# zhangxiaochen95/uav_bs_ctrl

Hardware: AMD Instinct MI355X
Metric: env-steps/sec (MADRQN, 8 UBS x 80 GT) (higher is better)
Workload: dtype f32

## Files before the change

### include/uavgnn.h

```cpp
#ifndef UAVGNN_H
#define UAVGNN_H

#include <stddef.h>
#include <stdint.h>

#ifdef __cplusplus
extern "C" {
#endif

#define UAVGNN_VERSION 100

#define UAVGNN_EINVAL (-1000)
#define UAVGNN_EUNSUPPORTED (-1001)
#define UAVGNN_EWORKSPACE (-1002)

typedef void* uavgnn_stream_t;

int uavgnn_version(void);

const char* uavgnn_strerror(int code);

int uavgnn_gatv2_fwd(const float* x_src, int E, int F_src, const float* x_dst, int F_dst, const int32_t* seg_off,
                     const int32_t* dst_order, int N, const float* W_s, const float* b_s, const float* W_d, const float* b_d, const float* attn,
                     const float* W_r, const float* b_r, int nh, int D, float slope, float* out, int ld_out,
// ... 72 lines not shown
                       int32_t* deg_near, uavgnn_stream_t stream);
int uavgnn_obs_compact(const float* gt, int M, int Fg, const float* ubs, int U, int Fu, int N, const int32_t* seen_off,
                       const int32_t* near_off, float* x_gt, float* x_ubs, uavgnn_stream_t stream);
int uavgnn_talk_degrees(const float* d_u2u, int n, int B, float r_comm, int32_t* deg_in, int32_t* env_edges,
                        uavgnn_stream_t stream);
int uavgnn_talk_compact(const float* d_u2u, int n, int B, float r_comm, const int32_t* talk_off,
                        const int32_t* env_base, int32_t* talk_src, int32_t* talk_eid, uavgnn_stream_t stream);
int uavgnn_offsets_scan4(const int32_t* d0, int n0, int32_t* o0, const int32_t* d1, int n1, int32_t* o1, const int32_t* d2,
                         int n2, int32_t* o2, const int32_t* d3, int n3, int32_t* o3, uavgnn_stream_t stream);

int uavgnn_eps_greedy(const float* q, int ld_q, int N, int A, int n_agents, const float* u_team, const float* u_agent,
                      float eps, long long* acts, uavgnn_stream_t stream);
int uavgnn_eps_greedy_dev(const float* q, int ld_q, int N, int A, int n_agents, const float* u_team, const float* u_agent,
                          const float* eps_dev, long long* acts, uavgnn_stream_t stream);

int uavgnn_colsum_acc(const float* x, long long ld, int N, int C, float* acc, int S, uavgnn_stream_t stream);
int uavgnn_gemm_h2_supported(int M, int N, int K);
long long uavgnn_split_h2_bytes(int n_out, int K);
int uavgnn_split_h2(const float* W, int ld, int R, int C, int transpose, void* planes, uavgnn_stream_t stream);
int uavgnn_gemm_nt_h2(const float* X, int ldx, int K1, const float* X2, int ldx2, int M, int K, const float* rowmax, const float* rowmax2,
                      const void* planes, int N, const float* bias, float* Y, int ldy, int epilogue, uavgnn_stream_t stream);
int uavgnn_gemm_nt_h2_rm2(const float* X, int ldx, int K1, const float* X2, int ldx2, int M, int K, const float* rowmax, float* rowmax2_out,
                          const void* planes, int N, const float* bias, float* Y, int ldy, int epilogue, uavgnn_stream_t stream);
int uavgnn_gru_gates_bwd_fused_sums_rowmax(const float* pre, const float* h, const float* d_hout, const float* dq, int n_out,
                                           const float* W_out, int N, int H, float* d_gi, float* d_gh, float* d_h, float* col_sums,
                                           float* row_absmax, uavgnn_stream_t stream);
int uavgnn_relu_bwd_colsum_rowmax(const float* dy, long long ld, const float* y, long long ldy, float* out, long long ldo, int N, int C,
                                  float* acc, int S, float* row_absmax, uavgnn_stream_t stream);
int uavgnn_relu_bwd_colsum(const float* dy, long long ld, const float* y, long long ldy, float* out, long long ldo, int N, int C,
                           float* acc, int S, uavgnn_stream_t stream);

int uavgnn_flat_obs_supported(int H_out, int F);
int uavgnn_flat_obs_fwd(const float* agent, long long ld_a, int F_a, const float* gt, long long ld_g, int K_g, const float* ubs,
                        long long ld_u, int K_u, int rows, const float* W, const float* b, int H_out, float* y, long long ld_y,
                        uavgnn_stream_t stream);
int uavgnn_flat_obs_wgrad_chunks(long long rows, int H_out, int F);
int uavgnn_flat_obs_wgrad(const float* dy, long long ld_dy, int H_out, const float* agent, long long ld_a, int F_a, const float* gt,
                          long long ld_g, int K_g, const float* ubs, long long ld_u, int K_u, int rows, float* partials, int S,
                          int accumulate, uavgnn_stream_t stream);

int uavgnn_talk_attn_env_supported(int n_max, int M, int K);
int uavgnn_talk_attn_env_fwd(const float* s, int ld_s, const float* q, int ld_q, const float* v, int ld_v, int K, int M,
                             const int32_t* talk_off, const int32_t* talk_src, const int32_t* graph_off, int B,
                             int n_max, float scale, float* c, int ld_c, float* a_save, const float* x_copy, int ld_x,
                             int n_copy, uavgnn_stream_t stream);
int uavgnn_talk_attn_env_bwd(const float* s, int ld_s, const float* q, int ld_q, const float* v, int ld_v, int K, int M,
// ... 123 lines not shown
```

### uav_bs_ctrl_amd/_lib.py

```python
from __future__ import annotations

import ctypes
import os

import torch as th

_HERE = os.path.dirname(os.path.abspath(__file__))
LIB_PATH = os.environ.get("UAVGNN_LIB") or os.path.join(_HERE, "csrc", "libuavgnn.so")

_c_fp = ctypes.c_void_p
_c_ip = ctypes.c_void_p
_c_int = ctypes.c_int
_c_f32 = ctypes.c_float
_c_st = ctypes.c_void_p

SIGNATURES = {
    "uavgnn_version": (_c_int, []),
    "uavgnn_strerror": (ctypes.c_char_p, [_c_int]),
    "uavgnn_gatv2_fwd": (_c_int, [_c_fp, _c_int, _c_int, _c_fp, _c_int, _c_ip, _c_ip, _c_int, _c_fp, _c_fp, _c_fp, _c_fp, _c_fp,
                                  _c_fp, _c_fp, _c_int, _c_int, _c_f32, _c_fp, _c_int, _c_fp, _c_st]),
    "uavgnn_gatv2_fwd_valu": (_c_int, [_c_fp, _c_int, _c_int, _c_fp, _c_int, _c_ip, _c_ip, _c_int, _c_fp, _c_fp, _c_fp, _c_fp, _c_fp,
                                       _c_fp, _c_fp, _c_int, _c_int, _c_f32, _c_fp, _c_int, _c_fp, _c_st]),
    "uavgnn_gatv2_fwd_mfma": (_c_int, [_c_fp, _c_int, _c_int, _c_fp, _c_int, _c_ip, _c_ip, _c_int, _c_fp, _c_fp, _c_fp, _c_fp, _c_fp,
                                       _c_fp, _c_fp, _c_int, _c_int, _c_f32, _c_fp, _c_int, _c_fp, _c_st]),
# ... 68 lines not shown
    "uavgnn_relu_bwd_colsum": (_c_int, [_c_fp, ctypes.c_longlong, _c_fp, ctypes.c_longlong, _c_fp, ctypes.c_longlong, _c_int, _c_int, _c_fp,
                               _c_int, _c_st]),
    "uavgnn_relu_bwd_colsum_rowmax": (_c_int, [_c_fp, ctypes.c_longlong, _c_fp, ctypes.c_longlong, _c_fp, ctypes.c_longlong, _c_int, _c_int,
                                               _c_fp, _c_int, _c_fp, _c_st]),
    "uavgnn_flat_obs_supported": (_c_int, [_c_int, _c_int]),
    "uavgnn_flat_obs_fwd": (_c_int, [_c_fp, ctypes.c_longlong, _c_int, _c_fp, ctypes.c_longlong, _c_int, _c_fp, ctypes.c_longlong, _c_int,
                                     _c_int, _c_fp, _c_fp, _c_int, _c_fp, ctypes.c_longlong, _c_st]),
    "uavgnn_flat_obs_wgrad_chunks": (_c_int, [ctypes.c_longlong, _c_int, _c_int]),
    "uavgnn_flat_obs_wgrad": (_c_int, [_c_fp, ctypes.c_longlong, _c_int, _c_fp, ctypes.c_longlong, _c_int, _c_fp, ctypes.c_longlong, _c_int,
                                       _c_fp, ctypes.c_longlong, _c_int, _c_int, _c_fp, _c_int, _c_int, _c_st]),
    "uavgnn_gemm_nt_x3_rowmax": (_c_int, [_c_fp, _c_int, _c_int, _c_int, ctypes.c_void_p, _c_int, _c_fp, _c_fp, _c_int, _c_int, _c_fp, _c_st]),
    "uavgnn_col_absmax": (_c_int, [_c_fp, ctypes.c_longlong, ctypes.c_longlong, _c_int, _c_fp, _c_st]),
    "uavgnn_gemm_tn_h2_supported": (_c_int, [ctypes.c_longlong, _c_int, _c_int]),
    "uavgnn_gemm_tn_h2_chunks": (_c_int, [ctypes.c_longlong, _c_int, _c_int]),
    "uavgnn_gemm_tn_h2": (_c_int, [_c_fp, ctypes.c_longlong, _c_int, _c_fp, ctypes.c_longlong, _c_int, ctypes.c_longlong, _c_fp, _c_fp, _c_fp,
                                   _c_int, _c_int, _c_st]),
    "uavgnn_gemm_h2_supported": (_c_int, [_c_int, _c_int, _c_int]),
    "uavgnn_split_h2_bytes": (ctypes.c_longlong, [_c_int, _c_int]),
    "uavgnn_split_h2": (_c_int, [_c_fp, _c_int, _c_int, _c_int, _c_int, ctypes.c_void_p, _c_st]),
    "uavgnn_gemm_nt_h2": (_c_int, [_c_fp, _c_int, _c_int, _c_fp, _c_int, _c_int, _c_int, _c_fp, _c_fp, ctypes.c_void_p, _c_int, _c_fp, _c_fp,
                                   _c_int, _c_int, _c_st]),
    "uavgnn_gemm_nt_h2_rm2": (_c_int, [_c_fp, _c_int, _c_int, _c_fp, _c_int, _c_int, _c_int, _c_fp, _c_fp, ctypes.c_void_p, _c_int, _c_fp, _c_fp,
                                       _c_int, _c_int, _c_st]),
    "uavgnn_env_state_dim": (_c_int, [_c_int, _c_int, _c_int]),
    "uavgnn_env_step": (_c_int, [ctypes.POINTER(ctypes.c_int32), ctypes.POINTER(ctypes.c_double), _c_int] + [_c_fp] * 22 + [_c_st]),
    "uavgnn_adamw_polyak": (_c_int, [_c_fp, _c_fp, _c_fp, _c_fp, _c_fp, ctypes.c_longlong, ctypes.c_longlong, _c_fp, ctypes.c_double,
                                     ctypes.c_double, _c_f32, _c_f32, _c_f32, _c_f32, _c_st]),
    "uavgnn_gru_cell_supported": (_c_int, [_c_int, _c_int]),
    "uavgnn_gru_cell_fwd": (_c_int, [_c_fp, _c_int, _c_int, _c_fp, _c_int, _c_int, _c_fp, _c_fp, _c_fp, _c_fp, _c_fp, _c_fp, _c_st]),
    "uavgnn_gru_cell_x3_supported": (_c_int, [_c_int, _c_int]),
    "uavgnn_gru_cell_x3_workspace_bytes": (ctypes.c_longlong, [_c_int, _c_int]),
    "uavgnn_gru_split_weights": (_c_int, [_c_fp, _c_int, _c_fp, _c_int, ctypes.c_void_p, _c_st]),
    "uavgnn_gru_cell_fwd_x3": (_c_int, [_c_fp, _c_int, _c_int, _c_fp, _c_int, _c_int, ctypes.c_void_p, _c_fp, _c_fp, _c_fp, _c_fp, _c_st]),
    "uavgnn_gru_cell_fwd_x3_cat": (_c_int, [_c_fp, _c_int, _c_int, _c_fp, _c_int, _c_int, _c_fp, _c_int, _c_int, ctypes.c_void_p, _c_fp, _c_fp,
                                            _c_fp, _c_fp, _c_st]),
    "uavgnn_gru_cell_fwd_x3_opts": (_c_int, [_c_fp, _c_int, _c_int, _c_fp, _c_int, _c_int, _c_fp, _c_int, _c_int, ctypes.c_void_p, _c_fp, _c_fp,
                                             _c_fp, _c_fp, _c_int, _c_st]),
    "uavgnn_gru_cell_h2_supported": (_c_int, [_c_int, _c_int]),
    "uavgnn_gru_cell_h2_workspace_bytes": (ctypes.c_longlong, [_c_int, _c_int]),
    "uavgnn_gru_split_weights_h2": (_c_int, [_c_fp, _c_int, _c_fp, _c_int, ctypes.c_void_p, _c_st]),
    "uavgnn_gru_cell_fwd_h2": (_c_int, [_c_fp, _c_int, _c_int, _c_fp, _c_int, _c_int, _c_fp, _c_int, _c_int, _c_fp, ctypes.c_void_p, _c_fp,
                                        _c_fp, _c_fp, _c_fp, _c_st]),
    "uavgnn_row_absmax": (_c_int, [_c_fp, _c_int, _c_int, _c_fp, _c_int, _c_int, _c_fp, _c_int, _c_int, _c_int, _c_fp, _c_st]),
    "uavgnn_tarmac_msg_rowmax_supported": (_c_int, [_c_int, _c_int, _c_int, _c_int]),
    "uavgnn_tarmac_msg_fwd_rowmax": (_c_int, [_c_fp, _c_int, _c_fp, _c_int, _c_int, _c_int, _c_int, ctypes.c_void_p, _c_fp, _c_int, _c_int,
                                              _c_ip, _c_ip, _c_f32, _c_fp, _c_int, _c_fp, _c_fp, _c_int, _c_fp, _c_int, _c_fp, _c_st]),
# ... 95 lines not shown
```

### uav_bs_ctrl_amd/csrc/gemm_h2.hip

```cpp
#include "common.h"

namespace uavgnn {
namespace {

typedef float f32x2 __attribute__((ext_vector_type(2)));
typedef float f32x16 __attribute__((ext_vector_type(16)));
typedef _Float16 f16x2 __attribute__((ext_vector_type(2)));
typedef _Float16 f16x8 __attribute__((ext_vector_type(8)));
typedef unsigned u32x4 __attribute__((ext_vector_type(4)));
typedef unsigned u32x2 __attribute__((ext_vector_type(2)));

constexpr int BN = 128, BK = 32, BM8 = 256, NT = 512;
constexpr int PA = BM8 * 4, PB = BN * 4;
constexpr int BUF = 2 * PA + 2 * PB;

__device__ __forceinline__ int swz32(int row) { return (row >> 2) & 3; }
__device__ __forceinline__ f16x8 as_frag(u32x4 v) { return __builtin_bit_cast(f16x8, v); }
__device__ __forceinline__ f32x16 mfma32(f16x8 a, f16x8 b, f32x16 c) { return __builtin_amdgcn_mfma_f32_32x32x16_f16(a, b, c, 0, 0, 0); }
__device__ __forceinline__ int scale_exp(float amax) {
  const int e = static_cast<int>((__float_as_uint(amax) >> 23) & 0xffu);
  return max(-126, min(126, 14 - (e - 127)));
}
__device__ __forceinline__ float pow2f(int e) { return __uint_as_float(static_cast<unsigned>(e + 127) << 23); }

// ... 286 lines not shown
    }
    return;
  }
  }
#pragma unroll
  for (int b = 0; b < 2; ++b) {
    const int col = n0 + wn + b * 32 + l32;
    if (col >= N) continue;
    const float bv = bias != nullptr ? bias[col] : 0.f, ci = winv[col];
#pragma unroll
    for (int a = 0; a < 2; ++a)
#pragma unroll
      for (int i = 0; i < 16; ++i) {
        const int lrow = wm + a * 32 + 8 * (i >> 2) + 4 * lh + (i & 3);
        const int row = m0 + lrow;
        if (row < M) {
          float* p = Y + static_cast<size_t>(row) * ldy + col;
          float v = acc[a][b][i] * ci * sInv[lrow] + bv;
          if (ACC) v += *p;
          if (RELU) v = fmaxf(v, 0.f);
          *p = v;
        }
      }
  }
}

}
}

using namespace uavgnn;

extern "C" int uavgnn_gemm_h2_supported(int M, int N, int K) {
  return (M > 0 && N > 0 && K >= BK && K % BK == 0 && static_cast<long long>(M) * K < (1LL << 31) &&
          2LL * N * K < (1LL << 31)) ? 1 : 0;
}

extern "C" long long uavgnn_split_h2_bytes(int n_out, int K) {
  if (n_out <= 0 || K <= 0) return 0;
  return 4LL * n_out * K + 4LL * n_out;
}

extern "C" int uavgnn_split_h2(const float* W, int ld, int R, int C, int transpose, void* planes, uavgnn_stream_t stream) {
  if (!W || !planes || R <= 0 || C <= 0 || ld < C) return UAVGNN_EINVAL;
  const int n_out = transpose ? C : R, K = transpose ? R : C;
  if ((K & 1) || (reinterpret_cast<uintptr_t>(planes) & 15)) return UAVGNN_EUNSUPPORTED;
  unsigned short* p = static_cast<unsigned short*>(planes);
// ... 29 lines not shown
  if (acc && relu) UAVGNN_H2_GEMM(true, true, IL);    \
  else if (acc) UAVGNN_H2_GEMM(true, false, IL);      \
  else if (relu) UAVGNN_H2_GEMM(false, true, IL);     \
  else UAVGNN_H2_GEMM(false, false, IL);
  if (epilogue & UAVGNN_GEMM_STAGING_INTERLEAVED) { UAVGNN_H2_GEMM_IL(true) }
  else { UAVGNN_H2_GEMM_IL(false) }
#undef UAVGNN_H2_GEMM_IL
#undef UAVGNN_H2_GEMM
  return launch_status();
}

extern "C" int uavgnn_gemm_nt_h2(const float* X, int ldx, int K1, const float* X2, int ldx2, int M, int K, const float* rowmax,
                                 const float* rowmax2, const void* planes, int N, const float* bias, float* Y, int ldy, int epilogue,
                                 uavgnn_stream_t stream) {
  return gemm_nt_h2_launch(X, ldx, K1, X2, ldx2, M, K, rowmax, rowmax2, nullptr, planes, N, bias, Y, ldy, epilogue, stream);
}

extern "C" int uavgnn_gemm_nt_h2_rm2(const float* X, int ldx, int K1, const float* X2, int ldx2, int M, int K, const float* rowmax,
                                     float* rowmax2_out, const void* planes, int N, const float* bias, float* Y, int ldy, int epilogue,
                                     uavgnn_stream_t stream) {
  if (!rowmax2_out) return UAVGNN_EINVAL;
  return gemm_nt_h2_launch(X, ldx, K1, X2, ldx2, M, K, rowmax, nullptr, rowmax2_out, planes, N, bias, Y, ldy, epilogue, stream);
}
```

### uav_bs_ctrl_amd/csrc/gru_fused.hip

```cpp
#include "common.h"

namespace uavgnn {
namespace {

typedef float f32x4 __attribute__((ext_vector_type(4)));
constexpr int BM = 128, BJ = 32, BK = 32, ST = 34;

__device__ __forceinline__ float sigmoidf_(float x) { return 1.f / (1.f + expf(-x)); }

template <bool SAVE>
__global__ __launch_bounds__(256, 2) void gru_cell_fwd_kernel(
    const float* __restrict__ inp, int ld_inp, int K1, const float* __restrict__ h, int N, int H,
    const float* __restrict__ W_ih, const float* __restrict__ b_ih, const float* __restrict__ W_hh,
    const float* __restrict__ b_hh, float* __restrict__ h_out, float* __restrict__ pre) {
  __shared__ __attribute__((aligned(16))) float sA[BM * ST];
  __shared__ __attribute__((aligned(16))) float sB[3 * BJ * ST];
  const int tid = threadIdx.x, lane = tid & 63, wave = tid >> 6;
  const int j = lane & 15, g = lane >> 4;
  const int wm = (wave >> 1) * 64, wc = (wave & 1) * 16;
  const int m0 = blockIdx.y * BM, j0 = blockIdx.x * BJ;

  f32x4 acc[4][4];
#pragma unroll
  for (int a = 0; a < 4; ++a)
// ... 99 lines not shown
      const float nn = tanhf(fmaf(rr, ghn, gin));
      float* hp = sA + lrow * ST + wc + j;
      *hp = fmaf(zz, *hp - nn, nn);
      if (SAVE && row < N) {
        float* p = pre + static_cast<size_t>(row) * 4 * H + c;
        p[0] = pr;
        p[H] = pz;
        p[2 * H] = gin;
        p[3 * H] = ghn;
      }
    }
  }
  __syncthreads();
#pragma unroll
  for (int q = 0; q < 4; ++q) {
    const int idx = tid + 256 * q, row = idx >> 3, c4 = idx & 7;
    if (m0 + row < N) {
      const float* p = sA + row * ST + 4 * c4;
      *reinterpret_cast<float4*>(h_out + static_cast<size_t>(m0 + row) * H + j0 + 4 * c4) = make_float4(p[0], p[1], p[2], p[3]);
    }
  }
}

template <bool HEAD, bool SUMS, bool RM = false>
__global__ __launch_bounds__(256) void gru_gates_bwd_fused_kernel(const float* __restrict__ pre, const float* __restrict__ h,
                                                                  const float* __restrict__ d_hout, long long total, int H,
                                                                  float* __restrict__ d_gi, float* __restrict__ d_gh,
                                                                  float* __restrict__ d_h, const float* __restrict__ dq,
                                                                  int n_out, const float* __restrict__ W_out,
                                                                  float* __restrict__ col_sums,
                                                                  float* __restrict__ row_absmax = nullptr) {
  const int HV = H / 4;
  float cs[SUMS ? 16 : 1];
#pragma unroll
  for (int t = 0; t < (SUMS ? 16 : 1); ++t) cs[t] = 0.f;
  for (long long i = blockIdx.x * 256LL + threadIdx.x; i < total; i += gridDim.x * 256LL) {
    const long long row = i / HV;
    const int col = static_cast<int>(i - row * HV) * 4;
    const float* p = pre + row * 4 * H + col;
    const float4 pr = *reinterpret_cast<const float4*>(p), pz = *reinterpret_cast<const float4*>(p + H);
    const float4 gin = *reinterpret_cast<const float4*>(p + 2 * H), ghn = *reinterpret_cast<const float4*>(p + 3 * H);
    const float4 hh = *reinterpret_cast<const float4*>(h + row * H + col);
    float4 dho = d_hout != nullptr ? *reinterpret_cast<const float4*>(d_hout + row * H + col) : make_float4(0.f, 0.f, 0.f, 0.f);
    if constexpr (HEAD) {
      const float* __restrict__ qr = dq + row * n_out;
      for (int a = 0; a < n_out; ++a) {
        const float qa = qr[a];
// ... 5 lines not shown
      }
    }
    const float a_pr[4] = {pr.x, pr.y, pr.z, pr.w}, a_pz[4] = {pz.x, pz.y, pz.z, pz.w};
    const float a_gi[4] = {gin.x, gin.y, gin.z, gin.w}, a_gh[4] = {ghn.x, ghn.y, ghn.z, ghn.w};
    const float a_h[4] = {hh.x, hh.y, hh.z, hh.w}, a_d[4] = {dho.x, dho.y, dho.z, dho.w};
    float dr[4], dz[4], dni[4], dnh[4], dh[4];
#pragma unroll
    for (int t = 0; t < 4; ++t) {
      const float r = sigmoidf_(a_pr[t]), z = sigmoidf_(a_pz[t]);
      const float n = tanhf(fmaf(r, a_gh[t], a_gi[t]));
      const float dn_pre = a_d[t] * (1.f - z) * (1.f - n * n);
      dni[t] = dn_pre;
      dnh[t] = dn_pre * r;
      dr[t] = dn_pre * a_gh[t] * r * (1.f - r);
      dz[t] = a_d[t] * (a_h[t] - n) * z * (1.f - z);
      dh[t] = a_d[t] * z;
      if constexpr (SUMS) {
        cs[t] += dr[t];
        cs[4 + t] += dz[t];
        cs[8 + t] += dni[t];
        cs[12 + t] += dnh[t];
      }
    }
    float* gi = d_gi + row * 3 * H + col;
    float* gh = d_gh + row * 3 * H + col;
    *reinterpret_cast<float4*>(gi) = make_float4(dr[0], dr[1], dr[2], dr[3]);
    *reinterpret_cast<float4*>(gi + H) = make_float4(dz[0], dz[1], dz[2], dz[3]);
    *reinterpret_cast<float4*>(gi + 2 * H) = make_float4(dni[0], dni[1], dni[2], dni[3]);
    *reinterpret_cast<float4*>(gh) = make_float4(dr[0], dr[1], dr[2], dr[3]);
    *reinterpret_cast<float4*>(gh + H) = make_float4(dz[0], dz[1], dz[2], dz[3]);
    *reinterpret_cast<float4*>(gh + 2 * H) = make_float4(dnh[0], dnh[1], dnh[2], dnh[3]);
    *reinterpret_cast<float4*>(d_h + row * H + col) = make_float4(dh[0], dh[1], dh[2], dh[3]);
    if constexpr (RM) {
      float m = 0.f;
#pragma unroll
      for (int t = 0; t < 4; ++t) m = fmaxf(fmaxf(fmaxf(m, fabsf(dr[t])), fmaxf(fabsf(dz[t]), fabsf(dni[t]))), fabsf(dnh[t]));
      m = wave_max(m);
      if ((threadIdx.x & 63) == 0) row_absmax[row] = m;
    }
  }
  if constexpr (SUMS) {
    __shared__ float sS[256 * 17];
#pragma unroll
    for (int t = 0; t < 16; ++t) sS[threadIdx.x * 17 + t] = cs[t];
    __syncthreads();
    if (static_cast<int>(threadIdx.x) < HV) {
      float* out = col_sums + static_cast<size_t>(blockIdx.x) * 4 * H + 4 * threadIdx.x;
#pragma unroll
      for (int gate = 0; gate < 4; ++gate) {
        float v[4];
#pragma unroll
        for (int t = 0; t < 4; ++t) {
          float a = 0.f;
          for (int part = threadIdx.x; part < 256; part += HV) a += sS[part * 17 + 4 * gate + t];
// ... 74 lines not shown
  const long long total = static_cast<long long>(N) * (H / 4);
  const dim3 grid(capped_grid(total, 256)), block(256);
  if (dq != nullptr)
    hipLaunchKernelGGL((gru_gates_bwd_fused_kernel<true, true>), grid, block, 0, static_cast<hipStream_t>(stream), pre, h, d_hout, total, H,
                       d_gi, d_gh, d_h, dq, n_out, W_out, col_sums);
  else
    hipLaunchKernelGGL((gru_gates_bwd_fused_kernel<false, true>), grid, block, 0, static_cast<hipStream_t>(stream), pre, h, d_hout, total, H,
                       d_gi, d_gh, d_h, nullptr, 0, nullptr, col_sums);
  return launch_status();
}

extern "C" int uavgnn_gru_gates_bwd_fused_sums_rowmax(const float* pre, const float* h, const float* d_hout, const float* dq, int n_out,
                                                      const float* W_out, int N, int H, float* d_gi, float* d_gh, float* d_h,
                                                      float* col_sums, float* row_absmax, uavgnn_stream_t stream) {
  if (N < 0 || H <= 0 || !pre || !h || !d_gi || !d_gh || !d_h || !col_sums || !row_absmax || (dq == nullptr) != (W_out == nullptr) ||
      (dq == nullptr && d_hout == nullptr) || (dq != nullptr && n_out <= 0))
    return UAVGNN_EINVAL;
  if (N == 0) return 0;
  if (H != 256 || !uavgnn_gru_gates_bwd_sum_rows(N, H) || n_out > 64 ||
      ((reinterpret_cast<uintptr_t>(W_out) | reinterpret_cast<uintptr_t>(col_sums)) & 15))
    return UAVGNN_EUNSUPPORTED;
  const long long total = static_cast<long long>(N) * (H / 4);
  const dim3 grid(capped_grid(total, 256)), block(256);
  if (dq != nullptr)
    hipLaunchKernelGGL((gru_gates_bwd_fused_kernel<true, true, true>), grid, block, 0, static_cast<hipStream_t>(stream), pre, h, d_hout, total,
                       H, d_gi, d_gh, d_h, dq, n_out, W_out, col_sums, row_absmax);
  else
    hipLaunchKernelGGL((gru_gates_bwd_fused_kernel<false, true, true>), grid, block, 0, static_cast<hipStream_t>(stream), pre, h, d_hout,
                       total, H, d_gi, d_gh, d_h, nullptr, 0, nullptr, col_sums, row_absmax);
  return launch_status();
}
```

### uav_bs_ctrl_amd/ops.py

```python
from __future__ import annotations

import os
import torch as th

from . import _lib as L

NEG_SLOPE = 0.2
K1_IMAGE = os.environ.get("UAVGNN_K1_IMAGE", "1") != "0"
HETERO_FUSED = True
K1_BF16Z = os.environ.get("UAVGNN_K1_BF16Z", "1") != "0"
K1_ROWMAX = os.environ.get("UAVGNN_K1_ROWMAX", "1") != "0"
K1_ROWMAX_MIN_ROWS = 1 << 17
GEMM_H2_RM2 = os.environ.get("UAVGNN_GEMM_H2_RM2", "1") != "0"
K1_ROWMAX_DENSE_DEG = int(os.environ.get("UAVGNN_K1_ROWMAX_DENSE_DEG", "16"))
K1_ROWMAX_DENSE_MIN_ROWS = 16384


class _KernelTimer:

    def __init__(self):
        self.enabled = False
        self.only = None
        self._spans = {}

# ... 628 lines not shown
            L.check(lib.uavgnn_split_h2(Wc.data_ptr(), n_out, K, n_out, 1, p.data_ptr(), L.stream()), "uavgnn_split_h2")
        keep = (W, W2)
    else:
        R, C = W.shape
        n_out, K = (C, R) if transpose_w else (R, C)
        assert K == K1 and W.stride(1) == 1
        key = ("h2mat", W.data_ptr(), W._version, W.stride(0), R, C, bool(transpose_w))

        def build(p):
            L.check(lib.uavgnn_split_h2(W.data_ptr(), W.stride(0), R, C, int(transpose_w), p.data_ptr(), L.stream()), "uavgnn_split_h2")
        keep = (W,)
    if out is None:
        out = th.empty((M, n_out), dtype=th.float32, device=a.device)
    with KERNEL_TIMER.span("gemm_h2", (M, n_out, K)):
        planes = _cached_planes(key, lib.uavgnn_split_h2_bytes(n_out, K), a.device, build, keep=keep)
        fn, rm2 = (lib.uavgnn_gemm_nt_h2, rowmax2) if rowmax2_out is None else (lib.uavgnn_gemm_nt_h2_rm2, rowmax2_out)
        rc = fn(a.data_ptr(), a.stride(0), K1, L.ptr(a2), 0 if a2 is None else a2.stride(0), M, K, rowmax.data_ptr(),
                L.ptr(rm2), planes.data_ptr(), n_out, L.ptr(bias), out.data_ptr(), out.stride(0),
                (1 if accumulate else 0) | (2 if relu else 0) | (GEMM_X3_FLAGS & 4), L.stream())
    L.check(rc, "uavgnn_gemm_nt_h2")
    return out


GEMM_TN_X3 = os.environ.get("UAVGNN_GEMM_TN_X3", "1") != "0"
GEMM_TN_MIN_ROWS = 1 << 18
GEMM_TN_H2 = os.environ.get("UAVGNN_GEMM_TN_H2", "1") != "0"


def _max_two_stage(t):
    n = t.numel()
    S = 1
    while S < 1024 and n % (2 * S) == 0 and n // (2 * S) >= 256:
        S *= 2
    return t.reshape(S, n // S).max(1).values.max()


def gemm_tn_h2_supported(dy, x, min_in=128) -> bool:
    return bool(GEMM_X3 and GEMM_H2 and GEMM_TN_H2 and dy.is_cuda and dy.dtype == th.float32 and x.dtype == th.float32 and dy.dim() == 2
                and x.dim() == 2 and dy.shape[0] == x.shape[0] and dy.shape[0] >= GEMM_TN_MIN_ROWS and dy.stride(1) == 1 and x.stride(1) == 1
                and dy.stride(0) % 4 == 0 and x.stride(0) % 4 == 0 and dy.data_ptr() % 16 == 0 and x.data_ptr() % 16 == 0
                and dy.shape[1] >= 256 and x.shape[1] >= min_in
                and L.lib().uavgnn_gemm_tn_h2_supported(dy.shape[0], dy.shape[1], x.shape[1]))


def gemm_tn_x3_supported(dy, x) -> bool:
    return bool(GEMM_X3 and GEMM_TN_X3 and dy.is_cuda and dy.dtype == th.float32 and x.dtype == th.float32 and dy.dim() == 2
# ... 251 lines not shown

    def bias(self, key, dy, flush_fn):
        n, C = dy.shape
        S = _row_blocks(n)
        key = (key, S)
        slot = self.slots.get(key)
        if slot is None:
            self.slots[key] = slot = (th.zeros((S, C), dtype=th.float32, device=dy.device), flush_fn)
        if dy.dtype != th.float32 or dy.stride(1) != 1:
            dy = dy.float().contiguous()
        L.check(L.lib().uavgnn_colsum_acc(dy.data_ptr(), dy.stride(0), n, C, slot[0].data_ptr(), S, L.stream()),
                "uavgnn_colsum_acc")

    def begin_sequence(self, T1, N, x_all):
        self.seq = _SequenceStage(T1, N, x_all.detach(), getattr(self, "_seq_bufs", None))
        self._seq_bufs = self.seq.bufs

    def end_sequence(self):
        seq, self.seq = getattr(self, "seq", None), None
        if seq is None or not seq.bwd_steps:
            return
        T1, N = seq.T1, seq.N
        full = sorted(seq.bwd_steps) == list(range(T1)) and seq.t_fwd == T1
        spans = [(0, T1)] if full else [(t, t + 1) for t in sorted(seq.bwd_steps)]
        split, ids, H = seq.split, seq.ids, seq.H
        for (t0, t1) in spans:
            rows = lambda name, lo=0: seq.bufs[name][t0 + lo:t1 + lo].reshape((t1 - t0) * N, -1)
            d_proj, d_gi, d_gh = rows("d_proj"), rows("d_gi"), rows("d_gh")
            dq = seq.dq_rows(t0, t1)
            x = seq.x_all[t0 * N:t1 * N]
            h, h2, inp = rows("h"), rows("h", 1), rows("inp")
            tn = False
            h2_bounds = full and seq.rowmax_steps >= set(range(T1)) and seq.rm_g_steps >= set(range(T1))
            if h2_bounds and seq.rm_p_steps >= set(range(T1)) and gemm_tn_h2_supported(x, d_proj, 96) and gemm_tn_h2_supported(h, d_proj, 96):
                bxh, bpj = _max_two_stage(seq.bufs["rowmax"][:T1]), _max_two_stage(seq.bufs["rm_p"][:T1])
                self.weight_h2(("Wp_x", ids["Wp"]), x, d_proj, bxh, bpj, lambda g: split("Wp", g.t(), 0))
                self.weight_h2(("Wp_h", ids["Wp"]), h, d_proj, bxh, bpj, lambda g: split("Wp", g.t(), H))
            else:
                self.weight(("Wp_x", ids["Wp"]), d_proj, x, lambda g: split("Wp", g, 0), tn)
                self.weight(("Wp_h", ids["Wp"]), d_proj, h, lambda g: split("Wp", g, H), tn)
            self.bias(("bp", ids["Wp"]), d_proj, lambda g: split("bp", g, 0))
            if h2_bounds and gemm_tn_h2_supported(d_gi, inp) and gemm_tn_h2_supported(d_gh, h):
                bx, by = _max_two_stage(seq.bufs["rowmax"][:T1]), _max_two_stage(seq.bufs["rm_g"][:T1])
                self.weight_h2(("W_ih", ids["W_ih"]), d_gi, inp, by, bx, lambda g: split("W_ih", g, 0))
                self.weight_h2(("W_hh", ids["W_hh"]), d_gh, h, by, bx, lambda g: split("W_hh", g, 0))
            else:
                self.weight(("W_ih", ids["W_ih"]), d_gi, inp, lambda g: split("W_ih", g, 0), tn)
                self.weight(("W_hh", ids["W_hh"]), d_gh, h, lambda g: split("W_hh", g, 0), tn)
            if all(t in seq.gsum_steps for t in range(t0, t1)):
                gs = seq.bufs["gsum"][t0:t1]
                gs = gs.reshape(gs.shape[0] * gs.shape[1], 4 * H)
                self.bias(("b_ih", ids["W_ih"]), gs[:, :3 * H], lambda g: split("b_ih", g, 0))
                self.bias(("b_hh_n", ids["W_hh"]), gs[:, 3 * H:], lambda g: split("b_hh", g, 2 * H))
            else:
                self.bias(("b_ih", ids["W_ih"]), d_gi, lambda g: split("b_ih", g, 0))
                self.bias(("b_hh_n", ids["W_hh"]), d_gh[:, 2 * H:], lambda g: split("b_hh", g, 2 * H))
            self.weight(("W_out", ids["W_out"]), dq, h2, lambda g: split("W_out", g, 0), tn)
            self.bias(("b_out", ids["W_out"]), dq, lambda g: split("b_out", g, 0))

    def flush(self):
        self.end_sequence()
        for key, (buf, fn) in self.slots.items():
            if fn is not None:
                fn(buf.sum(0))
        self.slots = {}
        self.owned.clear()
        self._seq_bufs = None


class _SequenceStage:

    def __init__(self, T1, N, x_all, bufs=None):
        self.T1, self.N, self.x_all = T1, N, x_all
        self.bufs = bufs if bufs is not None else {}
        self.t_fwd = 0
        self.bwd_steps = []
        self.gsum_steps = set()
        self.rowmax_steps = set()
        self.rm_g_steps = set()
        self.rm_p_steps = set()
        self.dq_steps = {}
        self.split = self.ids = self.H = None

    def dq_rows(self, t0, t1):
        parts = [self.dq_steps[t] for t in range(t0, t1)]
        if len(parts) == 1:
            return parts[0] if parts[0].is_contiguous() else parts[0].contiguous()
        first, (N, A) = parts[0], parts[0].shape
        if all(p.is_contiguous() and p.shape == (N, A) and p.dtype == first.dtype and
               p.untyped_storage().data_ptr() == first.untyped_storage().data_ptr() and
               p.storage_offset() == first.storage_offset() + i * N * A for i, p in enumerate(parts)):
            return first.as_strided(((t1 - t0) * N, A), (A, 1), first.storage_offset())
        return th.cat(parts, 0)

    def slot(self, name, t, cols, extra=0, rows=None):
        n = self.N if rows is None else rows
        b = self.bufs.get(name)
        if b is None or b.shape != (self.T1 + extra, n, cols) or b.device != self.x_all.device:
            b = self.bufs[name] = th.empty((self.T1 + extra, n, cols), dtype=th.float32, device=self.x_all.device)
        return b[t]


# ... 187 lines not shown
                h2 = th.empty_like(h)
                with KERNEL_TIMER.span("gru_gates_fwd"):
                    rc = L.lib().uavgnn_gru_gates_fwd(gi.data_ptr(), gh.data_ptr(), h.data_ptr(), N, H, h2.data_ptr(), L.stream())
                L.check(rc, "uavgnn_gru_gates_fwd")
        q = head_fwd(h2, W_out, b_out)
        if proj is None:
            proj = h2
        ctx.dims = (M, K)
        ctx.split, ctx.env, ctx.dx_out, ctx.fused_gru = split, env, dx_out, fused
        ctx.have_pre = bool(train) or not fused
        ctx.save_for_backward(x, h, proj, inp, gi, gh, h2, a_save, Wp, W_ih, W_hh, W_out, talk_off, talk_src, t_off,
                              t_dst, t_pos)
        return q, h2

    @staticmethod
    def backward(ctx, dq, dh2):
        (x, h, proj, inp, gi, gh, h2, a_save, Wp, W_ih, W_hh, W_out, talk_off, talk_src, t_off, t_dst,
         t_pos) = ctx.saved_tensors
        M, K = ctx.dims
        N, H = x.shape
        if not ctx.have_pre:
            raise L.UavGnnError("tarmac_step: backward through a forward that saved no pre-activations (train=False)")
        sink = GRAD_SINK
        rm_g = None
        dq = L.f32c(dq) if dq is not None else th.zeros((N, W_out.shape[0]), dtype=th.float32, device=x.device)
        head = None
        if (HEAD_FUSED_BWD and ctx.fused_gru and H % 4 == 0 and W_out.shape[0] <= 64 and W_out.is_contiguous()
                and W_out.dtype == th.float32 and W_out.data_ptr() % 16 == 0
                and (dh2 is None or (dh2.is_contiguous() and dh2.dtype == th.float32 and dh2.shape == (N, H)))):
            head = (dq, W_out.detach())
            dh2_tot = dh2
            if sink is not None:
                sink.owned.clear()
        elif dh2 is None:
            dh2_tot = th.mm(dq, W_out)
        elif (sink is not None and dh2.is_contiguous() and dh2.dtype == th.float32 and dh2.shape == (N, H)
              and sink.owned.get(dh2.data_ptr()) is not None):
            sink.owned.clear()
            dh2_tot = dh2.addmm_(dq, W_out)
        else:
            dh2_tot = th.addmm(dh2, dq, W_out)
        seq = ctx.seq if (sink is not None and ctx.seq is not None and sink.seq is ctx.seq) else None
        if seq is not None:
            t = ctx.seq_t
            G = L.lib().uavgnn_gru_gates_bwd_sum_rows(N, H) if GATE_SUMS else 0
            sums = None
            if G and (head is not None or dh2_tot is not None):
                sums = seq.slot("gsum", t, 4 * H, rows=G)
                seq.gsum_steps.add(t)
            rm_g = None
            if (sums is not None and H == 256 and W_hh.stride(1) == 1 and gemm_h2_supported(seq.slot("d_gh", t, 3 * H), H, 3 * H)):
                rm_g = seq.slot("rm_g", t, 1).view(N)
                seq.rm_g_steps.add(t)
            d_gi, d_gh, dh = _gru_gates_bwd_from_pre(gi, h, dh2_tot, seq.slot("d_gi", t, 3 * H), seq.slot("d_gh", t, 3 * H),
                                                     head=head, sums=sums, rowmax=rm_g)
        elif ctx.fused_gru:
            d_gi, d_gh, dh = _gru_gates_bwd_from_pre(gi, h, dh2_tot, head=head)
        else:
            d_gi, d_gh, dh = th.empty_like(gi), th.empty_like(gh), th.empty_like(h)
            with KERNEL_TIMER.span("gru_gates_bwd"):
                rc = L.lib().uavgnn_gru_gates_bwd(gi.data_ptr(), gh.data_ptr(), h.data_ptr(), dh2_tot.data_ptr(), N, H,
                                                  d_gi.data_ptr(), d_gh.data_ptr(), dh.data_ptr(), L.stream())
            L.check(rc, "uavgnn_gru_gates_bwd")
        split_dinp = (DINP_SPLIT and M > 0 and W_ih.stride(1) == 1 and gemm_x3_supported(d_gi, H, W_ih.shape[0])
                      and (ctx.dx_out is None or (ctx.dx_out.stride(1) == 1 and ctx.dx_out.dtype == th.float32)))
        ld = M + 2 * K
        d_proj = th.empty((N, ld), dtype=th.float32, device=x.device) if seq is None else seq.slot("d_proj", ctx.seq_t, ld)
        dx_cat = False
        if split_dinp:
            dx = ctx.dx_out if ctx.dx_out is not None else th.empty((N, H), dtype=th.float32, device=x.device)
            dx_cat = Wp.stride(1) == 1 and gemm_x3_cat_supported(d_gi, d_proj, H)
            if not dx_cat:
                _mm_nn(d_gi, W_ih[:, :H], out=dx)
            d_c = th.mm(d_gi, W_ih[:, H:])
            d_c_ptr, d_c_ld = d_c.data_ptr(), M
        else:
            d_inp = _mm_nn(d_gi, W_ih)
            d_c_ptr, d_c_ld = d_inp.data_ptr() + 4 * H, H + M
        _mm_nn(d_gh, W_hh, out=dh, accumulate=True, rowmax=rm_g)
        if sink is not None:
            sink.owned.clear()
            sink.owned[dh.data_ptr()] = dh
        _launch_talk_bwd(ctx.env, proj.data_ptr() + 4 * M, ld, proj.data_ptr() + 4 * (M + K), ld, proj.data_ptr(), ld,
                         K, M, talk_off, talk_src, (t_off, t_dst, t_pos), N, 1.0 / K, a_save, d_c_ptr,
                         d_c_ld, d_proj.data_ptr() + 4 * M, ld, d_proj.data_ptr() + 4 * (M + K), ld, d_proj.data_ptr(),
                         ld)
        if dx_cat and rm_g is not None and gemm_h2_supported(d_gi, H, d_gi.shape[1] + d_proj.shape[1]):
            if seq is not None:
                rm_p = seq.slot("rm_p", ctx.seq_t, 1).view(N)
                seq.rm_p_steps.add(ctx.seq_t)
            else:
                rm_p = th.empty(N, dtype=th.float32, device=d_gi.device)
            if GEMM_H2_RM2:
                gemm_h2(d_gi, W_ih[:, :H], rm_g, True, out=dx, a2=d_proj, W2=Wp[:, :H], rowmax2_out=rm_p)
            else:
                gemm_h2(d_gi, W_ih[:, :H], rm_g, True, out=dx, a2=d_proj, W2=Wp[:, :H], rowmax2=row_absmax(d_proj, out=rm_p))
        elif dx_cat:
            gemm_x3_cat(d_gi, d_proj, W_ih[:, :H], Wp[:, :H], dx)
        elif split_dinp:
            dx.addmm_(d_proj, Wp[:, :H])
        else:
            dx = ctx.dx_out
# ... 124 lines not shown
```

Before: 2.591 million.

## Pack GRU gate grads into shared g4 buffer and add N=64 split-half GEMM

The GRU backward kernel can now write its gate gradients into one packed [dnh, dr, dz, dni] buffer. d_gi and d_gh become overlapping views of it, which removes the duplicated r/z stores. The dh GEMM becomes a two-operand split-half GEMM over the packed layout, and the weight-gradient path reorders the W_hh rows to match. A new 128x64-tile split-half MFMA GEMM kernel replaces th.mm for the d_c product when M=64 and the grid is large enough. This adds a reduced-precision path and some layout-dependent bookkeeping.

```diff
diff --git a/include/uavgnn.h b/include/uavgnn.h
--- a/include/uavgnn.h
+++ b/include/uavgnn.h
@@ -118,6 +118,8 @@
                       const void* planes, int N, const float* bias, float* Y, int ldy, int epilogue, uavgnn_stream_t stream);
 int uavgnn_gemm_nt_h2_rm2(const float* X, int ldx, int K1, const float* X2, int ldx2, int M, int K, const float* rowmax, float* rowmax2_out,
                           const void* planes, int N, const float* bias, float* Y, int ldy, int epilogue, uavgnn_stream_t stream);
+int uavgnn_gemm_nt_h2_n64(const float* X, int ldx, int M, int K, const float* rowmax, const void* planes, int N, float* Y, int ldy,
+                          uavgnn_stream_t stream);
 int uavgnn_gru_gates_bwd_fused_sums_rowmax(const float* pre, const float* h, const float* d_hout, const float* dq, int n_out,
                                            const float* W_out, int N, int H, float* d_gi, float* d_gh, float* d_h, float* col_sums,
                                            float* row_absmax, uavgnn_stream_t stream);
diff --git a/uav_bs_ctrl_amd/_lib.py b/uav_bs_ctrl_amd/_lib.py
--- a/uav_bs_ctrl_amd/_lib.py
+++ b/uav_bs_ctrl_amd/_lib.py
@@ -114,6 +114,7 @@
                                    _c_int, _c_int, _c_st]),
     "uavgnn_gemm_nt_h2_rm2": (_c_int, [_c_fp, _c_int, _c_int, _c_fp, _c_int, _c_int, _c_int, _c_fp, _c_fp, ctypes.c_void_p, _c_int, _c_fp, _c_fp,
                                        _c_int, _c_int, _c_st]),
+    "uavgnn_gemm_nt_h2_n64": (_c_int, [_c_fp, _c_int, _c_int, _c_int, _c_fp, ctypes.c_void_p, _c_int, _c_fp, _c_int, _c_st]),
     "uavgnn_env_state_dim": (_c_int, [_c_int, _c_int, _c_int]),
     "uavgnn_env_step": (_c_int, [ctypes.POINTER(ctypes.c_int32), ctypes.POINTER(ctypes.c_double), _c_int] + [_c_fp] * 22 + [_c_st]),
     "uavgnn_adamw_polyak": (_c_int, [_c_fp, _c_fp, _c_fp, _c_fp, _c_fp, ctypes.c_longlong, ctypes.c_longlong, _c_fp, ctypes.c_double,
diff --git a/uav_bs_ctrl_amd/csrc/gemm_h2.hip b/uav_bs_ctrl_amd/csrc/gemm_h2.hip
--- a/uav_bs_ctrl_amd/csrc/gemm_h2.hip
+++ b/uav_bs_ctrl_amd/csrc/gemm_h2.hip
@@ -332,6 +332,127 @@
           *p = v;
         }
       }
+  }
+}
+
+constexpr int BM6 = 128, BN6 = 64;
+constexpr int PA6 = BM6 * 4, PB6 = BN6 * 4;
+constexpr int SUB6 = 2 * PA6 + 2 * PB6;
+constexpr int BUF6 = 2 * SUB6;
+
+__global__ __launch_bounds__(NT) void gemm_nt_h2n64_kernel(const float* __restrict__ X, int ldx, int M, int K,
+                                                           const unsigned short* __restrict__ Bp, int N, const float* __restrict__ winv,
+                                                           float* __restrict__ Y, int ldy, int col_blocks, const float* __restrict__ rm1) {
+  constexpr int LDT = BN6 + 4;
+  static_assert(BM6 * LDT * 4 <= 2 * BUF6 * 16, "the output tile fits the staging buffers");
+  __shared__ u32x4 smem[2 * BUF6];
+  __shared__ float sInv[BM6];
+  const int tid = threadIdx.x, lane = tid & 63, wave = tid >> 6;
+  const int l32 = lane & 31, lh = lane >> 5, sw = swz32(l32);
+  const int wm = (wave >> 1) * 32, wn = (wave & 1) * 32;
+  const int rb = blockIdx.x / col_blocks, cb = blockIdx.x - rb * col_blocks;
+  const int m0 = rb * BM6, n0 = cb * BN6;
+
+  f32x16 acc;
+#pragma unroll
+  for (int i = 0; i < 16; ++i) acc[i] = 0.f;
+
+  const int lr = tid >> 3, c4 = tid & 7;
+  unsigned xo[2];
+  float sca[2];
+#pragma unroll
+  for (int i = 0; i < 2; ++i) {
+    const int row = min(m0 + lr + 64 * i, M - 1);
+    xo[i] = static_cast<unsigned>(row) * ldx + 4 * c4;
+    sca[i] = pow2f(scale_exp(rm1[row]));
+  }
+  if (tid < BM6) sInv[tid] = pow2f(-scale_exp(rm1[min(m0 + tid, M - 1)]));
+  const int sa_w = lr * 32 + (((c4 >> 1) ^ swz32(lr)) * 8) + (c4 & 1) * 4;
+  const int bpl = tid >> 8, brow = (tid >> 2) & 63, bc = tid & 3;
+  const unsigned bo = bpl * (static_cast<unsigned>(N) * K) + static_cast<unsigned>(n0 + brow) * K + 8 * bc;
+  const int sbw = 2 * PA6 + bpl * PB6 + brow * 4 + (bc ^ swz32(brow));
+  const int ns = K / (2 * BK);
+  float4 ra[2][2];
+  u32x4 rw[2];
+  auto gload = [&](int t) {
+    const unsigned k0 = static_cast<unsigned>(min(t, ns - 1)) * (2 * BK);
+#pragma unroll
+    for (int s = 0; s < 2; ++s) {
+#pragma unroll
+      for (int i = 0; i < 2; ++i) ra[s][i] = *reinterpret_cast<const float4*>(X + (xo[i] + k0 + s * BK));
+      rw[s] = *reinterpret_cast<const u32x4*>(Bp + (bo + k0 + s * BK));
+    }
+  };
+  auto lstore = [&](int buf) {
+#pragma unroll
+    for (int s = 0; s < 2; ++s) {
+      u32x4* sb = smem + buf * BUF6 + s * SUB6;
+      unsigned short* sa = reinterpret_cast<unsigned short*>(sb) + sa_w;
+#pragma unroll
+      for (int i = 0; i < 2; ++i) stage4(sa + 64 * i * 32, PA6 * 8, ra[s][i], sca[i]);
+      sb[sbw] = rw[s];
+    }
+  };
+  struct Half {
+    f16x8 a[2], b[2];
+  };
+#define UAVGNN_N64_READ(F, buf, s, kh)                                                                     \
+  {                                                                                                        \
+    const u32x4* sb = smem + (buf) * BUF6 + (s) * SUB6;                                                    \
+    _Pragma("unroll") for (int pl = 0; pl < 2; ++pl) {                                                     \
+      F.a[pl] = as_frag(sb[pl * PA6 + (wm + l32) * 4 + ((2 * (kh) + lh) ^ sw)]);                           \
+      F.b[pl] = as_frag(sb[2 * PA6 + pl * PB6 + (wn + l32) * 4 + ((2 * (kh) + lh) ^ sw)]);                 \
+    }                                                                                                      \
+  }
+#define UAVGNN_N64_MFMA(F)                 \
+  {                                        \
+    acc = mfma32(F.a[0], F.b[1], acc);     \
+    acc = mfma32(F.a[1], F.b[0], acc);     \
+    acc = mfma32(F.a[0], F.b[0], acc);     \
+  }
+  gload(0);
+  lstore(0);
+  gload(1);
+  __syncthreads();
+  Half f0, f1, f2, f3;
+  UAVGNN_N64_READ(f0, 0, 0, 0)
+  for (int t = 0; t < ns; ++t) {
+    const int cur = t & 1;
+    UAVGNN_N64_READ(f1, cur, 0, 1)
+    lstore(cur ^ 1);
+    gload(t + 2);
+    __builtin_amdgcn_sched_barrier(0);
+    UAVGNN_N64_MFMA(f0)
+    UAVGNN_N64_READ(f2, cur, 1, 0)
+    UAVGNN_N64_MFMA(f1)
+    UAVGNN_N64_READ(f3, cur, 1, 1)
+    UAVGNN_N64_MFMA(f2)
+    __builtin_amdgcn_sched_barrier(0);
+    __syncthreads();
+    UAVGNN_N64_READ(f0, cur ^ 1, 0, 0)
+    __builtin_amdgcn_sched_barrier(0);
+    UAVGNN_N64_MFMA(f3)
+    __builtin_amdgcn_sched_barrier(0);
+  }
+#undef UAVGNN_N64_MFMA
+#undef UAVGNN_N64_READ
+  float* sT = reinterpret_cast<float*>(smem);
+  __syncthreads();
+  {
+    const float ci = winv[n0 + wn + l32];
+#pragma unroll
+    for (int i = 0; i < 16; ++i) {
+      const int lrow = wm + 8 * (i >> 2) + 4 * lh + (i & 3);
+      sT[lrow * LDT + wn + l32] = acc[i] * ci * sInv[lrow];
+    }
+  }
+  __syncthreads();
+#pragma unroll
+  for (int q = 0; q < 4; ++q) {
+    const int idx = tid + NT * q, row = idx >> 4, cc = idx & 15;
+    if (m0 + row < M)
+      *reinterpret_cast<float4*>(Y + static_cast<size_t>(m0 + row) * ldy + n0 + 4 * cc) =
+          *reinterpret_cast<const float4*>(sT + row * LDT + 4 * cc);
   }
 }
 
@@ -407,3 +528,18 @@
   if (!rowmax2_out) return UAVGNN_EINVAL;
   return gemm_nt_h2_launch(X, ldx, K1, X2, ldx2, M, K, rowmax, nullptr, rowmax2_out, planes, N, bias, Y, ldy, epilogue, stream);
 }
+
+extern "C" int uavgnn_gemm_nt_h2_n64(const float* X, int ldx, int M, int K, const float* rowmax, const void* planes, int N, float* Y,
+                                     int ldy, uavgnn_stream_t stream) {
+  if (M < 0 || !X || !planes || !Y || !rowmax || K <= 0 || N <= 0 || ldx < K || ldy < N) return UAVGNN_EINVAL;
+  if (M == 0) return 0;
+  if (!uavgnn_gemm_h2_supported(M, N, K) || (N % BN6) || (K % (2 * BK)) || (ldx & 3) || (ldy & 3) || static_cast<long long>(M) * ldx >= (1LL << 31) ||
+      ((reinterpret_cast<uintptr_t>(X) | reinterpret_cast<uintptr_t>(planes) | reinterpret_cast<uintptr_t>(Y)) & 15))
+    return UAVGNN_EUNSUPPORTED;
+  const unsigned short* bp = static_cast<const unsigned short*>(planes);
+  const float* winv = reinterpret_cast<const float*>(bp + 2LL * N * K);
+  const int col_blocks = N / BN6, row_blocks = (M + BM6 - 1) / BM6;
+  hipLaunchKernelGGL(gemm_nt_h2n64_kernel, dim3(row_blocks * col_blocks), dim3(NT), 0, static_cast<hipStream_t>(stream), X, ldx, M, K, bp,
+                     N, winv, Y, ldy, col_blocks, rowmax);
+  return launch_status();
+}
diff --git a/uav_bs_ctrl_amd/csrc/gru_fused.hip b/uav_bs_ctrl_amd/csrc/gru_fused.hip
--- a/uav_bs_ctrl_amd/csrc/gru_fused.hip
+++ b/uav_bs_ctrl_amd/csrc/gru_fused.hip
@@ -145,7 +145,7 @@
   }
 }
 
-template <bool HEAD, bool SUMS, bool RM = false>
+template <bool HEAD, bool SUMS, bool RM = false, bool PACK = false>
 __global__ __launch_bounds__(256) void gru_gates_bwd_fused_kernel(const float* __restrict__ pre, const float* __restrict__ h,
                                                                   const float* __restrict__ d_hout, long long total, int H,
                                                                   float* __restrict__ d_gi, float* __restrict__ d_gh,
@@ -197,14 +197,22 @@
         cs[12 + t] += dnh[t];
       }
     }
-    float* gi = d_gi + row * 3 * H + col;
-    float* gh = d_gh + row * 3 * H + col;
-    *reinterpret_cast<float4*>(gi) = make_float4(dr[0], dr[1], dr[2], dr[3]);
-    *reinterpret_cast<float4*>(gi + H) = make_float4(dz[0], dz[1], dz[2], dz[3]);
-    *reinterpret_cast<float4*>(gi + 2 * H) = make_float4(dni[0], dni[1], dni[2], dni[3]);
-    *reinterpret_cast<float4*>(gh) = make_float4(dr[0], dr[1], dr[2], dr[3]);
-    *reinterpret_cast<float4*>(gh + H) = make_float4(dz[0], dz[1], dz[2], dz[3]);
-    *reinterpret_cast<float4*>(gh + 2 * H) = make_float4(dnh[0], dnh[1], dnh[2], dnh[3]);
+    if constexpr (PACK) {
+      float* g4 = d_gh + row * 4 * H + col;
+      *reinterpret_cast<float4*>(g4) = make_float4(dnh[0], dnh[1], dnh[2], dnh[3]);
+      *reinterpret_cast<float4*>(g4 + H) = make_float4(dr[0], dr[1], dr[2], dr[3]);
+      *reinterpret_cast<float4*>(g4 + 2 * H) = make_float4(dz[0], dz[1], dz[2], dz[3]);
+      *reinterpret_cast<float4*>(g4 + 3 * H) = make_float4(dni[0], dni[1], dni[2], dni[3]);
+    } else {
+      float* gi = d_gi + row * 3 * H + col;
+      float* gh = d_gh + row * 3 * H + col;
+      *reinterpret_cast<float4*>(gi) = make_float4(dr[0], dr[1], dr[2], dr[3]);
+      *reinterpret_cast<float4*>(gi + H) = make_float4(dz[0], dz[1], dz[2], dz[3]);
+      *reinterpret_cast<float4*>(gi + 2 * H) = make_float4(dni[0], dni[1], dni[2], dni[3]);
+      *reinterpret_cast<float4*>(gh) = make_float4(dr[0], dr[1], dr[2], dr[3]);
+      *reinterpret_cast<float4*>(gh + H) = make_float4(dz[0], dz[1], dz[2], dz[3]);
+      *reinterpret_cast<float4*>(gh + 2 * H) = make_float4(dnh[0], dnh[1], dnh[2], dnh[3]);
+    }
     *reinterpret_cast<float4*>(d_h + row * H + col) = make_float4(dh[0], dh[1], dh[2], dh[3]);
     if constexpr (RM) {
       float m = 0.f;
@@ -325,6 +333,16 @@
     return UAVGNN_EUNSUPPORTED;
   const long long total = static_cast<long long>(N) * (H / 4);
   const dim3 grid(capped_grid(total, 256)), block(256);
+  if (d_gi == d_gh + H) {
+    if ((reinterpret_cast<uintptr_t>(d_gh) & 15)) return UAVGNN_EUNSUPPORTED;
+    if (dq != nullptr)
+      hipLaunchKernelGGL((gru_gates_bwd_fused_kernel<true, true, true, true>), grid, block, 0, static_cast<hipStream_t>(stream), pre, h, d_hout,
+                         total, H, nullptr, d_gh, d_h, dq, n_out, W_out, col_sums, row_absmax);
+    else
+      hipLaunchKernelGGL((gru_gates_bwd_fused_kernel<false, true, true, true>), grid, block, 0, static_cast<hipStream_t>(stream), pre, h,
+                         d_hout, total, H, nullptr, d_gh, d_h, nullptr, 0, nullptr, col_sums, row_absmax);
+    return launch_status();
+  }
   if (dq != nullptr)
     hipLaunchKernelGGL((gru_gates_bwd_fused_kernel<true, true, true>), grid, block, 0, static_cast<hipStream_t>(stream), pre, h, d_hout, total,
                        H, d_gi, d_gh, d_h, dq, n_out, W_out, col_sums, row_absmax);
diff --git a/uav_bs_ctrl_amd/ops.py b/uav_bs_ctrl_amd/ops.py
--- a/uav_bs_ctrl_amd/ops.py
+++ b/uav_bs_ctrl_amd/ops.py
@@ -674,6 +674,35 @@
     return out
 
 
+G4 = os.environ.get("UAVGNN_G4", "1") != "0"
+DC_H2 = os.environ.get("UAVGNN_DC_H2", "1") != "0"
+GEMM_H2_N64_MIN_GRID = 128
+
+
+def gemm_h2_n64_supported(a, n_out, k) -> bool:
+    return bool(DC_H2 and GEMM_H2 and a.is_cuda and a.dtype == th.float32 and a.dim() == 2 and a.stride(1) == 1 and a.shape[1] == k
+                and a.stride(0) % 4 == 0 and a.data_ptr() % 16 == 0 and n_out % 64 == 0 and k % 64 == 0 and a.shape[0] * a.stride(0) < 2 ** 31
+                and L.lib().uavgnn_gemm_h2_supported(a.shape[0], n_out, k)
+                and ((a.shape[0] + 127) // 128) * (n_out // 64) >= GEMM_H2_N64_MIN_GRID)
+
+
+def gemm_h2_n64(a, W, rowmax, out=None):
+    lib = L.lib()
+    M, K = a.shape
+    R, n_out = W.shape
+    assert R == K and W.stride(1) == 1
+    if out is None:
+        out = th.empty((M, n_out), dtype=th.float32, device=a.device)
+    with KERNEL_TIMER.span("gemm_h2_n64", (M, n_out, K)):
+        planes = _cached_planes(("h2mat", W.data_ptr(), W._version, W.stride(0), R, n_out, True), lib.uavgnn_split_h2_bytes(n_out, K),
+                                a.device, lambda p: L.check(lib.uavgnn_split_h2(W.data_ptr(), W.stride(0), R, n_out, 1, p.data_ptr(),
+                                                                                 L.stream()), "uavgnn_split_h2"), keep=(W,))
+        rc = lib.uavgnn_gemm_nt_h2_n64(a.data_ptr(), a.stride(0), M, K, rowmax.data_ptr(), planes.data_ptr(), n_out, out.data_ptr(),
+                                       out.stride(0), L.stream())
+    L.check(rc, "uavgnn_gemm_nt_h2_n64")
+    return out
+
+
 GEMM_TN_X3 = os.environ.get("UAVGNN_GEMM_TN_X3", "1") != "0"
 GEMM_TN_MIN_ROWS = 1 << 18
 GEMM_TN_H2 = os.environ.get("UAVGNN_GEMM_TN_H2", "1") != "0"
@@ -971,11 +1000,20 @@
             return
         T1, N = seq.T1, seq.N
         full = sorted(seq.bwd_steps) == list(range(T1)) and seq.t_fwd == T1
+        if full and 0 < len(seq.g4_steps) < T1:
+            full = False
         spans = [(0, T1)] if full else [(t, t + 1) for t in sorted(seq.bwd_steps)]
         split, ids, H = seq.split, seq.ids, seq.H
         for (t0, t1) in spans:
             rows = lambda name, lo=0: seq.bufs[name][t0 + lo:t1 + lo].reshape((t1 - t0) * N, -1)
-            d_proj, d_gi, d_gh = rows("d_proj"), rows("d_gi"), rows("d_gh")
+            d_proj = rows("d_proj")
+            g4 = t0 in seq.g4_steps
+            if g4:
+                d_gi, d_gh = rows("g4")[:, H:], rows("g4")[:, :3 * H]
+                whh_key, whh_flush = "W_hh_nrz", lambda g: split("W_hh", th.cat((g[H:], g[:H]), 0), 0)
+            else:
+                d_gi, d_gh = rows("d_gi"), rows("d_gh")
+                whh_key, whh_flush = "W_hh", lambda g: split("W_hh", g, 0)
             dq = seq.dq_rows(t0, t1)
             x = seq.x_all[t0 * N:t1 * N]
             h, h2, inp = rows("h"), rows("h", 1), rows("inp")
@@ -992,10 +1030,10 @@
             if h2_bounds and gemm_tn_h2_supported(d_gi, inp) and gemm_tn_h2_supported(d_gh, h):
                 bx, by = _max_two_stage(seq.bufs["rowmax"][:T1]), _max_two_stage(seq.bufs["rm_g"][:T1])
                 self.weight_h2(("W_ih", ids["W_ih"]), d_gi, inp, by, bx, lambda g: split("W_ih", g, 0))
-                self.weight_h2(("W_hh", ids["W_hh"]), d_gh, h, by, bx, lambda g: split("W_hh", g, 0))
+                self.weight_h2((whh_key, ids["W_hh"]), d_gh, h, by, bx, whh_flush)
             else:
                 self.weight(("W_ih", ids["W_ih"]), d_gi, inp, lambda g: split("W_ih", g, 0), tn)
-                self.weight(("W_hh", ids["W_hh"]), d_gh, h, lambda g: split("W_hh", g, 0), tn)
+                self.weight((whh_key, ids["W_hh"]), d_gh, h, whh_flush, tn)
             if all(t in seq.gsum_steps for t in range(t0, t1)):
                 gs = seq.bufs["gsum"][t0:t1]
                 gs = gs.reshape(gs.shape[0] * gs.shape[1], 4 * H)
@@ -1003,7 +1041,7 @@
                 self.bias(("b_hh_n", ids["W_hh"]), gs[:, 3 * H:], lambda g: split("b_hh", g, 2 * H))
             else:
                 self.bias(("b_ih", ids["W_ih"]), d_gi, lambda g: split("b_ih", g, 0))
-                self.bias(("b_hh_n", ids["W_hh"]), d_gh[:, 2 * H:], lambda g: split("b_hh", g, 2 * H))
+                self.bias(("b_hh_n", ids["W_hh"]), d_gh[:, :H] if g4 else d_gh[:, 2 * H:], lambda g: split("b_hh", g, 2 * H))
             self.weight(("W_out", ids["W_out"]), dq, h2, lambda g: split("W_out", g, 0), tn)
             self.bias(("b_out", ids["W_out"]), dq, lambda g: split("b_out", g, 0))
 
@@ -1027,6 +1065,7 @@
         self.gsum_steps = set()
         self.rowmax_steps = set()
         self.rm_g_steps = set()
+        self.g4_steps = set()
         self.rm_p_steps = set()
         self.dq_steps = {}
         self.split = self.ids = self.H = None
@@ -1260,7 +1299,7 @@
         if not ctx.have_pre:
             raise L.UavGnnError("tarmac_step: backward through a forward that saved no pre-activations (train=False)")
         sink = GRAD_SINK
-        rm_g = None
+        rm_g = g4 = None
         dq = L.f32c(dq) if dq is not None else th.zeros((N, W_out.shape[0]), dtype=th.float32, device=x.device)
         head = None
         if (HEAD_FUSED_BWD and ctx.fused_gru and H % 4 == 0 and W_out.shape[0] <= 64 and W_out.is_contiguous()
@@ -1287,11 +1326,19 @@
                 sums = seq.slot("gsum", t, 4 * H, rows=G)
                 seq.gsum_steps.add(t)
             rm_g = None
-            if (sums is not None and H == 256 and W_hh.stride(1) == 1 and gemm_h2_supported(seq.slot("d_gh", t, 3 * H), H, 3 * H)):
-                rm_g = seq.slot("rm_g", t, 1).view(N)
-                seq.rm_g_steps.add(t)
-            d_gi, d_gh, dh = _gru_gates_bwd_from_pre(gi, h, dh2_tot, seq.slot("d_gi", t, 3 * H), seq.slot("d_gh", t, 3 * H),
-                                                     head=head, sums=sums, rowmax=rm_g)
+            if sums is not None and H == 256 and W_hh.stride(1) == 1:
+                if G4 and gemm_h2_supported(seq.slot("g4", t, 4 * H)[:, H:], H, 3 * H):
+                    g4 = seq.slot("g4", t, 4 * H)
+                    seq.g4_steps.add(t)
+                if g4 is not None or gemm_h2_supported(seq.slot("d_gh", t, 3 * H), H, 3 * H):
+                    rm_g = seq.slot("rm_g", t, 1).view(N)
+                    seq.rm_g_steps.add(t)
+            if g4 is not None:
+                d_gi, _, dh = _gru_gates_bwd_from_pre(gi, h, dh2_tot, g4[:, H:], g4[:, :3 * H], head=head, sums=sums, rowmax=rm_g)
+                d_gh = None
+            else:
+                d_gi, d_gh, dh = _gru_gates_bwd_from_pre(gi, h, dh2_tot, seq.slot("d_gi", t, 3 * H), seq.slot("d_gh", t, 3 * H),
+                                                         head=head, sums=sums, rowmax=rm_g)
         elif ctx.fused_gru:
             d_gi, d_gh, dh = _gru_gates_bwd_from_pre(gi, h, dh2_tot, head=head)
         else:
@@ -1310,12 +1357,18 @@
             dx_cat = Wp.stride(1) == 1 and gemm_x3_cat_supported(d_gi, d_proj, H)
             if not dx_cat:
                 _mm_nn(d_gi, W_ih[:, :H], out=dx)
-            d_c = th.mm(d_gi, W_ih[:, H:])
+            if rm_g is not None and M == 64 and gemm_h2_n64_supported(d_gi, M, 3 * H):
+                d_c = gemm_h2_n64(d_gi, W_ih[:, H:], rm_g)
+            else:
+                d_c = th.mm(d_gi, W_ih[:, H:])
             d_c_ptr, d_c_ld = d_c.data_ptr(), M
         else:
             d_inp = _mm_nn(d_gi, W_ih)
             d_c_ptr, d_c_ld = d_inp.data_ptr() + 4 * H, H + M
-        _mm_nn(d_gh, W_hh, out=dh, accumulate=True, rowmax=rm_g)
+        if g4 is not None:
+            gemm_h2(g4[:, H:3 * H], W_hh[:2 * H], rm_g, True, out=dh, accumulate=True, a2=g4[:, :H], W2=W_hh[2 * H:])
+        else:
+            _mm_nn(d_gh, W_hh, out=dh, accumulate=True, rowmax=rm_g)
         if sink is not None:
             sink.owned.clear()
             sink.owned[dh.data_ptr()] = dh
```

After: 2.623 million, median of 6. 1.2% higher.
